# Jittor/PointCloudLib

Hardware: AMD Instinct MI355X
Metric: point-clouds/sec fwd+bwd, PointNet++ SSG B=32 N=1024 (higher is better)
Workload: dtype f32; 1 GPU; PointNet++ SSG cls train step (fwd+bwd+SGD), B=32/GPU, N=1024 xyz+normal, gauss_ball clouds (BASELINE configs[1]); global_batch=32, n_points=1024, parallelism=dp1, launch=eager, grad_overlap=False, cpu_affinity=numa node 0 (gpu0), 128 cpus, world_size=1, sync_bn=False, entry_points=per-stack (pcl_mlp_stack_*_f32)

## Files before the change

### pointcloudlib_amd/csrc/compact.hip

```cpp
#include "common.h"

namespace pcl {

struct GoffMulti { const int32_t* cnt[4]; int32_t* goff[4]; };
__device__ __forceinline__ void group_offsets_body(const int32_t* __restrict__ cnt, int G, int32_t* __restrict__ goff);
__global__ __launch_bounds__(1024) void group_offsets_kernel(const int32_t* __restrict__ cnt, int G, int32_t* __restrict__ goff) {
    group_offsets_body(cnt, G, goff);
}
__global__ __launch_bounds__(1024) void group_offsets_multi_kernel(const GoffMulti a, int G) {
    group_offsets_body(a.cnt[blockIdx.x], G, a.goff[blockIdx.x]);
}
__device__ __forceinline__ void group_offsets_body(const int32_t* __restrict__ cnt, int G, int32_t* __restrict__ goff) {
    __shared__ int tot[16];
    constexpr int U = 8;
    const int lane = threadIdx.x & 63, w = threadIdx.x >> 6;
    const int per = ((G + 15) / 16 + 63) / 64 * 64;
    const int lo = min(w * per, G), hi = min(lo + per, G);
    int s = 0;
    rows_in_flight<U>(cnt, 1, lo + lane, 64, hi, [&](int, int v) { s += max(v, 1); });
#pragma unroll
    for (int o = 32; o > 0; o >>= 1) s += __shfl_xor(s, o);
    if (lane == 0) tot[w] = s;
    __syncthreads();
    int run = 0, all = 0;
#pragma unroll
    for (int j = 0; j < 16; ++j) { const int t = tot[j]; run += j < w ? t : 0; all += t; }
    rows_in_flight<U>(lo, 64, hi, [&](int g0) { return max(cnt[min(g0 + lane, hi - 1)], 1); },
                      [&](int g0, int v) {
                          int inc = v;
#pragma unroll
                          for (int o = 1; o < 64; o <<= 1) { const int t = __shfl_up(inc, o); if (lane >= o) inc += t; }
                          if (g0 + lane < hi) goff[g0 + lane] = run + inc - v;
                          run += __shfl(inc, 63);
                      });
    if (threadIdx.x == 0) goff[G] = all;
}

__global__ __launch_bounds__(256) void group_compact_kernel(const float* __restrict__ xyz, const float* __restrict__ new_xyz,
                                                            const float* __restrict__ feat, const int32_t* __restrict__ idx,
                                                            const int32_t* __restrict__ cnt, const int32_t* __restrict__ goff,
                                                            int G, int N, int m, int ns, int C, int use_xyz, int S,
                                                            float* __restrict__ rows, int2* __restrict__ rmeta,
                                                            int32_t* __restrict__ rsrc) {
    const int g = blockIdx.x, wave = threadIdx.x >> 6, lane = threadIdx.x & 63;
    const int D = (use_xyz ? 3 : 0) + C, off3 = use_xyz ? 3 : 0;
    const int c = max(cnt[g], 1), base = goff[g];
    const int b = g / m;
    const int32_t* I = idx + (size_t)g * ns;
    const int chunk = (ns + 3) >> 2;
    const int s_lo = wave * chunk, s_hi = min(s_lo + chunk, c);
    if (s_lo >= s_hi) return;
    float* o = rows + (size_t)base * S;
    const float* fb = feat ? feat + (size_t)b * N * C : nullptr;
    if (C >= 32) {
        float q[3] = {0.f, 0.f, 0.f};
        if (use_xyz && lane < 3) q[0] = new_xyz[(size_t)g * 3 + lane];
        for (int s = s_lo; s < s_hi; s += 4) {
            int k[4];
#pragma unroll
            for (int j = 0; j < 4; ++j) k[j] = I[min(s + j, s_hi - 1)];
            for (int c0 = 0; c0 < C; c0 += 128) {
                float v[4][2];
#pragma unroll
                for (int j = 0; j < 4; ++j)
#pragma unroll
                    for (int h = 0; h < 2; ++h) {
                        const int ch = min(c0 + h * 64 + lane, C - 1);
                        v[j][h] = fb[(size_t)k[j] * C + ch];
                    }
#pragma unroll
                for (int j = 0; j < 4; ++j)
#pragma unroll
                    for (int h = 0; h < 2; ++h) {
                        const int ch = c0 + h * 64 + lane;
                        if (s + j < s_hi && ch < C) o[(size_t)(s + j) * S + off3 + ch] = v[j][h];
                    }
            }
            if (use_xyz && lane < 3) {
#pragma unroll
                for (int j = 0; j < 4; ++j)
                    if (s + j < s_hi) o[(size_t)(s + j) * S + lane] = __fsub_rn(xyz[((size_t)b * N + k[j]) * 3 + lane], q[0]);
            }
            if (lane < S - D) {
#pragma unroll
                for (int j = 0; j < 4; ++j)
                    if (s + j < s_hi) o[(size_t)(s + j) * S + D + lane] = 0.f;
            }
        }
    } else {
        for (int s = s_lo + lane; s < s_hi; s += 64) {
            const int k = I[s];
            float* oo = o + (size_t)s * S;
            if (use_xyz) {
#pragma unroll
                for (int d = 0; d < 3; ++d) oo[d] = __fsub_rn(xyz[((size_t)b * N + k) * 3 + d], new_xyz[(size_t)g * 3 + d]);
            }
            for (int d = 0; d < C; ++d) oo[off3 + d] = fb[(size_t)k * C + d];
            for (int d = D; d < S; ++d) oo[d] = 0.f;
        }
    }
    for (int s = s_lo + lane; s < s_hi; s += 64) {
        const int mult = s == 0 ? ns - c + 1 : 1;
        rmeta[base + s] = make_int2(g, s | (mult << 16));
        rsrc[base + s] = b * N + I[s];
    }
}

template <int V>
__global__ __launch_bounds__(256) void bn_act_max_rows_kernel(const float* __restrict__ Y, const int32_t* __restrict__ goff,
                                                              const float* __restrict__ scale, const float* __restrict__ shift,
                                                              float slope, int G, int C, float* __restrict__ out,
                                                              int32_t* __restrict__ arg, float* __restrict__ ymax) {
    const int CV = C / V;
    const size_t total = (size_t)G * CV;
    for (size_t e = (size_t)blockIdx.x * 256 + threadIdx.x; e < total; e += (size_t)gridDim.x * 256) {
        const size_t g = e / CV;
        const int c = (int)(e - g * CV) * V;
        float a[V], bsh[V], best[V], by[V];
        int bi[V];
#pragma unroll
        for (int v = 0; v < V; ++v) { a[v] = scale[c + v]; bsh[v] = shift[c + v]; best[v] = -INFINITY; by[v] = 0.f; bi[v] = 0; }
        const int r0 = goff[g], r1 = goff[g + 1];
        for (int r = r0; r < r1; r += 4) {
            float yy[4][V];
#pragma unroll
            for (int j = 0; j < 4; ++j) {
                const float* src = Y + (size_t)min(r + j, r1 - 1) * C + c;
                if constexpr (V == 4) {
                    const float4 t = *reinterpret_cast<const float4*>(src);
                    yy[j][0] = t.x; yy[j][1] = t.y; yy[j][2] = t.z; yy[j][3] = t.w;
                } else {
                    yy[j][0] = *src;
                }
            }
#pragma unroll
            for (int j = 0; j < 4; ++j) {
                if (r + j < r1) {
#pragma unroll
                    for (int v = 0; v < V; ++v) {
                        const float u = fmaf(a[v], yy[j][v], bsh[v]);
                        const float z = u > 0.f ? u : u * slope;
                        if (z > best[v]) { best[v] = z; bi[v] = r + j - r0; by[v] = yy[j][v]; }
                    }
                }
            }
        }
#pragma unroll
        for (int v = 0; v < V; ++v) { out[g * C + c + v] = best[v]; arg[g * C + c + v] = bi[v]; ymax[g * C + c + v] = by[v]; }
    }
}

__global__ __launch_bounds__(256) void scatter_rows_add_kernel(const float* __restrict__ grows, const int32_t* __restrict__ rsrc,
                                                               const int32_t* __restrict__ n_rows, int D, int off, int C,
                                                               float* __restrict__ gfeat) {
    const int n = *n_rows, lane = threadIdx.x & 63;
    const int wv = blockIdx.x * 4 + (threadIdx.x >> 6), nw = gridDim.x * 4;
    for (int r = wv * 2; r < n; r += nw * 2) {
        const int r2 = min(r + 1, n - 1);
        const size_t d0 = (size_t)rsrc[r] * C, d1 = (size_t)rsrc[r2] * C;
        for (int c = lane; c < C; c += 64) {
            const float v0 = grows[(size_t)r * D + off + c], v1 = grows[(size_t)r2 * D + off + c];
            unsafeAtomicAdd(&gfeat[d0 + c], v0);
            if (r + 1 < n) unsafeAtomicAdd(&gfeat[d1 + c], v1);
        }
    }
}

constexpr int GL_MAXH = 4;
constexpr int GL_RPI = 4;
constexpr int GL_CF = 4;

__device__ __forceinline__ float glin_row_value(float u, const float4& L, const float4& F, const float (&wx)[3], const float (&wf)[GL_CF]) {
    const float t = fmaf(wx[2], L.z, fmaf(wx[1], L.y, fmaf(wx[0], L.x, u)));
    return fmaf(wf[3], F.w, fmaf(wf[2], F.z, fmaf(wf[1], F.y, fmaf(wf[0], F.x, t))));
}

struct DenseJob { const float* src; float* dst; int rows, cols, ldw, first, blocks; };

__global__ __launch_bounds__(256) void group_rows_meta_kernel(const float* __restrict__ xyz, const float* __restrict__ new_xyz,
                                                              const float* __restrict__ fs, int CF,
                                                              const int32_t* __restrict__ idx, const int32_t* __restrict__ cnt,
                                                              const int32_t* __restrict__ goff, int G, int N, int m, int ns,
                                                              int2* __restrict__ rmeta, int32_t* __restrict__ rsrc,
                                                              float4* __restrict__ rloc, float4* __restrict__ rfeat, DenseJob dj) {
    if ((int)blockIdx.x >= dj.first) {
        const int n = dj.rows * dj.cols;
        for (int i = ((int)blockIdx.x - dj.first) * 256 + (int)threadIdx.x; i < n; i += dj.blocks * 256) {
            const int r = i / dj.cols;
            dj.dst[i] = dj.src[(size_t)r * dj.ldw + (i - r * dj.cols)];
        }
        return;
    }
    const int g = blockIdx.x * 4 + (threadIdx.x >> 6), lane = threadIdx.x & 63;
    if (g >= G) return;
    const int c = max(cnt[g], 1), base = goff[g], b = g / m;
    const int32_t* I = idx + (size_t)g * ns;
    float q0 = 0.f, q1 = 0.f, q2 = 0.f;
    if (xyz) { q0 = new_xyz[(size_t)g * 3]; q1 = new_xyz[(size_t)g * 3 + 1]; q2 = new_xyz[(size_t)g * 3 + 2]; }
    for (int s = lane; s < c; s += 64) {
        const int mult = s == 0 ? ns - c + 1 : 1;
        const int src = b * N + I[s];
        rmeta[base + s] = make_int2(g, s | (mult << 16));
        rsrc[base + s] = src;
        float4 L = make_float4(0.f, 0.f, 0.f, (float)mult);
        if (xyz) {
            const float* pk = xyz + (size_t)src * 3;
            L.x = __fsub_rn(pk[0], q0); L.y = __fsub_rn(pk[1], q1); L.z = __fsub_rn(pk[2], q2);
        }
        rloc[base + s] = L;
        if (rfeat) {
            float f[4] = {0.f, 0.f, 0.f, 0.f};
            for (int j = 0; j < CF; ++j) f[j] = fs[(size_t)src * CF + j];
            rfeat[base + s] = make_float4(f[0], f[1], f[2], f[3]);
        }
    }
}

template <int NH>
__global__ __launch_bounds__(256) void group_linear_kernel(const float* __restrict__ Uf, const float* __restrict__ Wx,
                                                           const float* __restrict__ Wfs, int CF, int ldw,
                                                           const float4* __restrict__ rloc, const float4* __restrict__ rfeat,
                                                           const int32_t* __restrict__ rsrc,
                                                           const int32_t* __restrict__ n_rows, int C1, float* __restrict__ Y,
                                                           double* __restrict__ stats) {
    __shared__ double red[2][4][64 * NH];
    const int wave = threadIdx.x >> 6, lane = threadIdx.x & 63;
    const int R = *n_rows;
    float wx[NH][3], wf[NH][GL_CF];
    double ss[NH], qq[NH];
#pragma unroll
    for (int h = 0; h < NH; ++h) {
        const int ch = lane + 64 * h;
#pragma unroll
        for (int d = 0; d < 3; ++d) wx[h][d] = (Wx && ch < C1) ? Wx[(size_t)ch * ldw + d] : 0.f;
#pragma unroll
        for (int f = 0; f < GL_CF; ++f) wf[h][f] = (f < CF && ch < C1) ? Wfs[(size_t)ch * ldw + f] : 0.f;
        ss[h] = 0.0; qq[h] = 0.0;
    }
    const int stride = gridDim.x * 4 * GL_RPI;
    int r0 = (blockIdx.x * 4 + wave) * GL_RPI;
    float4 nl[GL_RPI], nf[GL_RPI]; int sr[GL_RPI];
#pragma unroll
    for (int j = 0; j < GL_RPI; ++j) {
        const int r = min(r0 + j, R - 1);
        nl[j] = rloc[r]; sr[j] = Uf ? rsrc[r] : 0; nf[j] = CF ? rfeat[r] : make_float4(0.f, 0.f, 0.f, 0.f);
    }
    for (; r0 < R; r0 += stride) {
        float4 L[GL_RPI], F[GL_RPI]; int cs[GL_RPI];
#pragma unroll
        for (int j = 0; j < GL_RPI; ++j) { L[j] = nl[j]; F[j] = nf[j]; cs[j] = sr[j]; }
        {
            const int rn = r0 + stride;
#pragma unroll
            for (int j = 0; j < GL_RPI; ++j) {
                const int r = min(rn + j, R - 1);
                nl[j] = rloc[r]; sr[j] = Uf ? rsrc[r] : 0; nf[j] = CF ? rfeat[r] : make_float4(0.f, 0.f, 0.f, 0.f);
            }
        }
#pragma unroll
        for (int h = 0; h < NH; ++h) {
            const int ch = min(lane + 64 * h, C1 - 1);
            float u[GL_RPI];
#pragma unroll
            for (int j = 0; j < GL_RPI; ++j) u[j] = Uf ? Uf[(size_t)cs[j] * C1 + ch] : 0.f;
#pragma unroll
            for (int j = 0; j < GL_RPI; ++j) {
                if (r0 + j < R && lane + 64 * h < C1) {
                    const float y = glin_row_value(u[j], L[j], F[j], wx[h], wf[h]);
                    Y[(size_t)(r0 + j) * C1 + ch] = y;
                    const double w = (double)L[j].w;
                    ss[h] += w * (double)y; qq[h] += w * (double)y * (double)y;
                }
            }
        }
    }
#pragma unroll
    for (int h = 0; h < NH; ++h) { red[0][wave][lane + 64 * h] = ss[h]; red[1][wave][lane + 64 * h] = qq[h]; }
    __syncthreads();
    for (int ch = threadIdx.x; ch < C1; ch += 256) {
        double* dst = stats + (size_t)blockIdx.x * 2 * C1;
        dst[ch] = (red[0][0][ch] + red[0][1][ch]) + (red[0][2][ch] + red[0][3][ch]);
        dst[C1 + ch] = (red[1][0][ch] + red[1][1][ch]) + (red[1][2][ch] + red[1][3][ch]);
    }
}

template <int NH>
__global__ __launch_bounds__(256) void group_linear_bwd_kernel(const float4* __restrict__ rloc, const float4* __restrict__ rfeat,
                                                               int CF, const float* __restrict__ dU, const float* __restrict__ Y,
                                                               const float* __restrict__ a_, const float* __restrict__ k1_,
                                                               const float* __restrict__ k2_, const float* __restrict__ mu_,
                                                               const int32_t* __restrict__ rsrc,
                                                               const int32_t* __restrict__ n_rows, int C1, float* __restrict__ dUf,
                                                               float* __restrict__ dWx_part, float* __restrict__ dWf_part) {
    __shared__ float red[3 + GL_CF][4][64 * NH];
    const int wave = threadIdx.x >> 6, lane = threadIdx.x & 63;
    const int R = *n_rows;
    float a[NH], k1[NH], k2[NH], mu[NH], gw[NH][3 + GL_CF];
#pragma unroll
    for (int h = 0; h < NH; ++h) {
        const int ch = min(lane + 64 * h, C1 - 1);
        a[h] = a_[ch]; k1[h] = k1_[ch]; k2[h] = k2_[ch]; mu[h] = mu_[ch];
#pragma unroll
        for (int d = 0; d < 3 + GL_CF; ++d) gw[h][d] = 0.f;
    }
    const int stride = gridDim.x * 4 * GL_RPI;
    int r0 = (blockIdx.x * 4 + wave) * GL_RPI;
    float4 nl[GL_RPI], nf[GL_RPI]; int sr[GL_RPI];
#pragma unroll
    for (int j = 0; j < GL_RPI; ++j) {
        const int r = min(r0 + j, R - 1);
        nl[j] = rloc[r]; sr[j] = dUf ? rsrc[r] : 0; nf[j] = dWf_part ? rfeat[r] : make_float4(0.f, 0.f, 0.f, 0.f);
    }
    for (; r0 < R; r0 += stride) {
        float4 L[GL_RPI], F[GL_RPI]; int cs[GL_RPI];
#pragma unroll
        for (int j = 0; j < GL_RPI; ++j) { L[j] = nl[j]; F[j] = nf[j]; cs[j] = sr[j]; }
        {
            const int rn = r0 + stride;
#pragma unroll
            for (int j = 0; j < GL_RPI; ++j) {
                const int r = min(rn + j, R - 1);
                nl[j] = rloc[r]; sr[j] = dUf ? rsrc[r] : 0; nf[j] = dWf_part ? rfeat[r] : make_float4(0.f, 0.f, 0.f, 0.f);
            }
        }
#pragma unroll
        for (int h = 0; h < NH; ++h) {
            const int ch = min(lane + 64 * h, C1 - 1);
            float du[GL_RPI], y[GL_RPI];
#pragma unroll
            for (int j = 0; j < GL_RPI; ++j) {
                const size_t o = (size_t)min(r0 + j, R - 1) * C1 + ch;
                du[j] = dU[o]; y[j] = Y[o];
            }
#pragma unroll
            for (int j = 0; j < GL_RPI; ++j) {
                if (r0 + j < R && lane + 64 * h < C1) {
                    const float dy = fmaf(a[h], du[j], -L[j].w * fmaf(k2[h], y[j] - mu[h], k1[h]));
                    if (dUf) unsafeAtomicAdd(&dUf[(size_t)cs[j] * C1 + ch], dy);
                    gw[h][0] = fmaf(dy, L[j].x, gw[h][0]); gw[h][1] = fmaf(dy, L[j].y, gw[h][1]);
                    gw[h][2] = fmaf(dy, L[j].z, gw[h][2]);
                    gw[h][3] = fmaf(dy, F[j].x, gw[h][3]); gw[h][4] = fmaf(dy, F[j].y, gw[h][4]);
                    gw[h][5] = fmaf(dy, F[j].z, gw[h][5]); gw[h][6] = fmaf(dy, F[j].w, gw[h][6]);
                }
            }
        }
    }
    if (dWx_part || dWf_part) {
#pragma unroll
        for (int h = 0; h < NH; ++h)
#pragma unroll
            for (int d = 0; d < 3 + GL_CF; ++d) red[d][wave][lane + 64 * h] = gw[h][d];
        __syncthreads();
        if (dWx_part)
            for (int e = threadIdx.x; e < C1 * 3; e += 256) {
                const int ch = e / 3, d = e - ch * 3;
                dWx_part[(size_t)blockIdx.x * C1 * 3 + e] = (red[d][0][ch] + red[d][1][ch]) + (red[d][2][ch] + red[d][3][ch]);
            }
        if (dWf_part)
            for (int e = threadIdx.x; e < C1 * CF; e += 256) {
                const int ch = e / CF, d = 3 + (e - ch * CF);
                dWf_part[(size_t)blockIdx.x * C1 * CF + e] = (red[d][0][ch] + red[d][1][ch]) + (red[d][2][ch] + red[d][3][ch]);
            }
    }
}

__device__ __forceinline__ void glin_load_weights(const float* __restrict__ Wx, const float* __restrict__ Wfs, int CF, int ldw, int c4,
                                                  float (&wx)[4][3], float (&wf)[4][GL_CF]) {
#pragma unroll
    for (int v = 0; v < 4; ++v) {
#pragma unroll
        for (int d = 0; d < 3; ++d) wx[v][d] = Wx ? Wx[(size_t)(c4 + v) * ldw + d] : 0.f;
#pragma unroll
        for (int f = 0; f < GL_CF; ++f) wf[v][f] = f < CF ? Wfs[(size_t)(c4 + v) * ldw + f] : 0.f;
    }
}
template <int LPR>
__global__ __launch_bounds__(256) void group_linear_v4_kernel(const float* __restrict__ Uf, const float* __restrict__ Wx,
                                                              const float* __restrict__ Wfs, int CF, int ldw,
                                                              const float4* __restrict__ rloc, const float4* __restrict__ rfeat,
                                                              const int32_t* __restrict__ rsrc,
                                                              const int32_t* __restrict__ n_rows, float* __restrict__ Y,
                                                              double* __restrict__ stats) {
    constexpr int C1 = 4 * LPR, RPW = 64 / LPR, U = 4;
    __shared__ double red[2][4][C1];
    const int wave = threadIdx.x >> 6, lane = threadIdx.x & 63;
    const int cl = lane % LPR, rsub = lane / LPR, c4 = 4 * cl;
    const int R = *n_rows;
    float wx[4][3], wf[4][GL_CF];
    double ss[4], qq[4];
#pragma unroll
    for (int v = 0; v < 4; ++v) {
#pragma unroll
        for (int d = 0; d < 3; ++d) wx[v][d] = Wx ? Wx[(size_t)(c4 + v) * ldw + d] : 0.f;
#pragma unroll
        for (int f = 0; f < GL_CF; ++f) wf[v][f] = f < CF ? Wfs[(size_t)(c4 + v) * ldw + f] : 0.f;
        ss[v] = 0.0; qq[v] = 0.0;
    }
    const int stride = gridDim.x * 4 * RPW * U;
    for (int r0 = (blockIdx.x * 4 + wave) * RPW * U; r0 < R; r0 += stride) {
        float4 L[U], F[U], u[U];
#pragma unroll
        for (int j = 0; j < U; ++j) {
            const int r = min(r0 + j * RPW + rsub, R - 1);
            L[j] = rloc[r];
            F[j] = CF ? rfeat[r] : make_float4(0.f, 0.f, 0.f, 0.f);
            u[j] = Uf ? *reinterpret_cast<const float4*>(Uf + (size_t)rsrc[r] * C1 + c4) : make_float4(0.f, 0.f, 0.f, 0.f);
        }
#pragma unroll
        for (int j = 0; j < U; ++j) {
            const int r = r0 + j * RPW + rsub;
            if (r < R) {
                float y[4] = {u[j].x, u[j].y, u[j].z, u[j].w};
                const double w = (double)L[j].w;
#pragma unroll
                for (int v = 0; v < 4; ++v) {
                    const float t = glin_row_value(y[v], L[j], F[j], wx[v], wf[v]);
                    y[v] = t;
                    ss[v] += w * (double)t; qq[v] += w * (double)t * (double)t;
                }
                *reinterpret_cast<float4*>(Y + (size_t)r * C1 + c4) = make_float4(y[0], y[1], y[2], y[3]);
            }
        }
    }
#pragma unroll
    for (int v = 0; v < 4; ++v) {
#pragma unroll
        for (int off = LPR; off < 64; off <<= 1) { ss[v] += __shfl_xor(ss[v], off); qq[v] += __shfl_xor(qq[v], off); }
        if (rsub == 0) { red[0][wave][c4 + v] = ss[v]; red[1][wave][c4 + v] = qq[v]; }
    }
    __syncthreads();
    for (int ch = threadIdx.x; ch < C1; ch += 256) {
        double* dst = stats + (size_t)blockIdx.x * 2 * C1;
        dst[ch] = (red[0][0][ch] + red[0][1][ch]) + (red[0][2][ch] + red[0][3][ch]);
        dst[C1 + ch] = (red[1][0][ch] + red[1][1][ch]) + (red[1][2][ch] + red[1][3][ch]);
    }
}

template <int LPR>
__global__ __launch_bounds__(256) void group_linear_bwd_v4_kernel(const float4* __restrict__ rloc, const float4* __restrict__ rfeat,
                                                                  int CF, const float* __restrict__ dU, const float* __restrict__ Y,
                                                                  const float* __restrict__ a_, const float* __restrict__ k1_,
                                                                  const float* __restrict__ k2_, const float* __restrict__ mu_,
                                                                  const int32_t* __restrict__ rsrc,
                                                                  const int32_t* __restrict__ n_rows, float* __restrict__ dUf,
                                                                  float* __restrict__ dWx_part, float* __restrict__ dWf_part) {
    constexpr int C1 = 4 * LPR, RPW = 64 / LPR, U = 4;
    __shared__ float red[3 + GL_CF][4][C1];
    const int wave = threadIdx.x >> 6, lane = threadIdx.x & 63;
    const int cl = lane % LPR, rsub = lane / LPR, c4 = 4 * cl;
    const int R = *n_rows;
    float a[4], k1[4], k2[4], mu[4], gw[3 + GL_CF][4];
#pragma unroll
    for (int v = 0; v < 4; ++v) {
        a[v] = a_[c4 + v]; k1[v] = k1_[c4 + v]; k2[v] = k2_[c4 + v]; mu[v] = mu_[c4 + v];
#pragma unroll
        for (int d = 0; d < 3 + GL_CF; ++d) gw[d][v] = 0.f;
    }
    const int stride = gridDim.x * 4 * RPW * U;
    for (int r0 = (blockIdx.x * 4 + wave) * RPW * U; r0 < R; r0 += stride) {
        float4 L[U], F[U], du[U], yv[U];
        int src[U];
#pragma unroll
        for (int j = 0; j < U; ++j) {
            const int r = min(r0 + j * RPW + rsub, R - 1);
            L[j] = rloc[r];
            F[j] = dWf_part ? rfeat[r] : make_float4(0.f, 0.f, 0.f, 0.f);
            src[j] = dUf ? rsrc[r] : 0;
            du[j] = *reinterpret_cast<const float4*>(dU + (size_t)r * C1 + c4);
            yv[j] = *reinterpret_cast<const float4*>(Y + (size_t)r * C1 + c4);
        }
#pragma unroll
        for (int j = 0; j < U; ++j) {
            const int r = r0 + j * RPW + rsub;
            if (r < R) {
                const float dd[4] = {du[j].x, du[j].y, du[j].z, du[j].w}, yy[4] = {yv[j].x, yv[j].y, yv[j].z, yv[j].w};
#pragma unroll
                for (int v = 0; v < 4; ++v) {
                    const float dy = fmaf(a[v], dd[v], -L[j].w * fmaf(k2[v], yy[v] - mu[v], k1[v]));
                    if (dUf) unsafeAtomicAdd(&dUf[(size_t)src[j] * C1 + c4 + v], dy);
                    gw[0][v] = fmaf(dy, L[j].x, gw[0][v]); gw[1][v] = fmaf(dy, L[j].y, gw[1][v]); gw[2][v] = fmaf(dy, L[j].z, gw[2][v]);
                    gw[3][v] = fmaf(dy, F[j].x, gw[3][v]); gw[4][v] = fmaf(dy, F[j].y, gw[4][v]);
                    gw[5][v] = fmaf(dy, F[j].z, gw[5][v]); gw[6][v] = fmaf(dy, F[j].w, gw[6][v]);
                }
            }
        }
    }
    if (dWx_part || dWf_part) {
#pragma unroll
        for (int d = 0; d < 3 + GL_CF; ++d)
#pragma unroll
            for (int v = 0; v < 4; ++v) {
                float t = gw[d][v];
#pragma unroll
                for (int off = LPR; off < 64; off <<= 1) t += __shfl_xor(t, off);
                if (rsub == 0) red[d][wave][c4 + v] = t;
            }
        __syncthreads();
        if (dWx_part)
            for (int e = threadIdx.x; e < C1 * 3; e += 256) {
                const int ch = e / 3, d = e - ch * 3;
                dWx_part[(size_t)blockIdx.x * C1 * 3 + e] = (red[d][0][ch] + red[d][1][ch]) + (red[d][2][ch] + red[d][3][ch]);
            }
        if (dWf_part)
            for (int e = threadIdx.x; e < C1 * CF; e += 256) {
                const int ch = e / CF, d = 3 + (e - ch * CF);
                dWf_part[(size_t)blockIdx.x * C1 * CF + e] = (red[d][0][ch] + red[d][1][ch]) + (red[d][2][ch] + red[d][3][ch]);
            }
    }
}

template <int LPR>
__global__ __launch_bounds__(256) void group_linear_bwd_regen_kernel(const float4* __restrict__ rloc, const float4* __restrict__ rfeat,
                                                                     const float* __restrict__ Wx, const float* __restrict__ Wfs, int CF,
                                                                     int ldw, const float* __restrict__ dU, const float* __restrict__ a_,
                                                                     const float* __restrict__ k1_, const float* __restrict__ k2_,
                                                                     const float* __restrict__ mu_, const int32_t* __restrict__ n_rows,
                                                                     float* __restrict__ dWx_part, float* __restrict__ dWf_part) {
    constexpr int C1 = 4 * LPR, RPW = 64 / LPR, CH = 4, U = 3;
    __shared__ float red[3 + GL_CF][4][C1];
    const int wave = threadIdx.x >> 6, lane = threadIdx.x & 63;
    const int cl = lane % LPR, rsub = lane / LPR, c4 = 4 * cl;
    const int R = *n_rows;
    float wx[4][3], wf[4][GL_CF];
    float a[4], k1[4], k2[4], mu[4], gw[3 + GL_CF][4];
    glin_load_weights(Wx, Wfs, CF, ldw, c4, wx, wf);
#pragma unroll
    for (int v = 0; v < 4; ++v) {
        a[v] = a_[c4 + v]; k1[v] = k1_[c4 + v]; k2[v] = k2_[c4 + v]; mu[v] = mu_[c4 + v];
#pragma unroll
        for (int d = 0; d < 3 + GL_CF; ++d) gw[d][v] = 0.f;
    }
    const int stride = gridDim.x * 4 * RPW * CH, base = (blockIdx.x * 4 + wave) * RPW * CH;
    for (int t0 = 0; base + (t0 / CH) * stride < R; t0 += U) {
        float4 L[U], F[U], du[U];
        int row[U];
#pragma unroll
        for (int j = 0; j < U; ++j) {
            const int t = t0 + j;
            row[j] = base + (t / CH) * stride + (t % CH) * RPW + rsub;
            const int r = min(row[j], R - 1);
            L[j] = rloc[r];
            F[j] = CF ? rfeat[r] : make_float4(0.f, 0.f, 0.f, 0.f);
            du[j] = *reinterpret_cast<const float4*>(dU + (size_t)r * C1 + c4);
        }
#pragma unroll
        for (int j = 0; j < U; ++j) {
            if (row[j] < R) {
                const float dd[4] = {du[j].x, du[j].y, du[j].z, du[j].w};
#pragma unroll
                for (int v = 0; v < 4; ++v) {
                    const float y = glin_row_value(0.f, L[j], F[j], wx[v], wf[v]);
                    const float dy = fmaf(a[v], dd[v], -L[j].w * fmaf(k2[v], y - mu[v], k1[v]));
                    gw[0][v] = fmaf(dy, L[j].x, gw[0][v]); gw[1][v] = fmaf(dy, L[j].y, gw[1][v]); gw[2][v] = fmaf(dy, L[j].z, gw[2][v]);
                    gw[3][v] = fmaf(dy, F[j].x, gw[3][v]); gw[4][v] = fmaf(dy, F[j].y, gw[4][v]);
                    gw[5][v] = fmaf(dy, F[j].z, gw[5][v]); gw[6][v] = fmaf(dy, F[j].w, gw[6][v]);
                }
            }
        }
    }
#pragma unroll
    for (int d = 0; d < 3 + GL_CF; ++d)
#pragma unroll
        for (int v = 0; v < 4; ++v) {
            float t = gw[d][v];
#pragma unroll
            for (int off = LPR; off < 64; off <<= 1) t += __shfl_xor(t, off);
            if (rsub == 0) red[d][wave][c4 + v] = t;
        }
    __syncthreads();
    if (dWx_part)
        for (int e = threadIdx.x; e < C1 * 3; e += 256) {
            const int ch = e / 3, d = e - ch * 3;
            dWx_part[(size_t)blockIdx.x * C1 * 3 + e] = (red[d][0][ch] + red[d][1][ch]) + (red[d][2][ch] + red[d][3][ch]);
        }
// ... 192 lines not shown
    __syncthreads();
    int run = inc - s;
    for (int w = 0; w < wave; ++w) run += wtot[w];
    for (int i = i0; i < i1; ++i) {
        const int t = off[i];
        off[i] = run;
        int pos = run;
        for (int w = 0; w < RT_W; ++w) { const int c = cnt[w * N + i]; cnt[w * N + i] = pos; pos += c; }
        run += t;
    }
    if (tid == 0) off[N] = re - rb;
    __syncthreads();
    for (int g = g0; g < g1; ++g) {
        const int q0 = group_off[g_first + g], q1 = group_off[g_first + g + 1];
        for (int r = q0 + lane; r < q1; r += 64) lst[atomicAdd(&mycnt[rsrc[r] - pbase], 1)] = r;
        __builtin_amdgcn_fence(__ATOMIC_SEQ_CST, "wavefront");
        __builtin_amdgcn_wave_barrier();
    }
    __syncthreads();
    for (int pl = tid; pl < N; pl += RT_T) in_off[pbase + pl] = rb + off[pl];
    if (b == B - 1 && tid == 0) in_off[pbase + N] = re;
    for (int i = tid; i < re - rb; i += RT_T) in_rows[rb + i] = lst[i];
}

__global__ __launch_bounds__(256) void group_linear_dw_kernel(const float* __restrict__ px, const float* __restrict__ pf, int rows,
                                                              int C1, int CF, int off, int ld, float* __restrict__ dW0) {
    const int nx = px ? C1 * 3 : 0, nf = pf ? C1 * CF : 0;
    const int e = blockIdx.x * 4 + (threadIdx.x >> 6), lane = threadIdx.x & 63;
    if (e >= nx + nf) return;
    const bool isx = e < nx;
    const float* src = isx ? px + e : pf + (e - nx);
    const int n = isx ? nx : nf;
    float s = 0.f;
    rows_in_flight<8>(src, n, lane, 64, rows, [&](int, float v) { s += v; });
#pragma unroll
    for (int o = 32; o > 0; o >>= 1) s += __shfl_xor(s, o);
    if (lane == 0) {
        if (isx) dW0[(size_t)(e / 3) * ld + e % 3] = s;
        else dW0[(size_t)((e - nx) / CF) * ld + off + (e - nx) % CF] = s;
    }
}

}
using namespace pcl;

extern "C" int pcl_group_offsets_i32(const int32_t* cnt, int G, int32_t* group_off, void* stream) {
    PCL_REQUIRE(cnt && group_off && G >= 1, "pcl_group_offsets_i32: bad arguments");
    hipLaunchKernelGGL(group_offsets_kernel, dim3(1), dim3(1024), 0, as_stream(stream), cnt, G, group_off);
    return check_launch("pcl_group_offsets_i32");
}

extern "C" int pcl_group_offsets_multi_i32(int n, const int32_t* const* cnt, int G, int32_t* const* group_off, void* stream) {
    PCL_REQUIRE(cnt && group_off && G >= 1 && n >= 1 && n <= 4, "pcl_group_offsets_multi_i32: bad arguments (n = %d: 1..4)", n);
    GoffMulti a = {};
    for (int i = 0; i < n; ++i) {
        PCL_REQUIRE(cnt[i] && group_off[i], "pcl_group_offsets_multi_i32: null array %d", i);
        a.cnt[i] = cnt[i]; a.goff[i] = group_off[i];
    }
    hipLaunchKernelGGL(group_offsets_multi_kernel, dim3(n), dim3(1024), 0, as_stream(stream), a, G);
    return check_launch("pcl_group_offsets_multi_i32");
}

extern "C" int pcl_group_compact_f32(const float* xyz, const float* new_xyz, const float* feat, const int32_t* idx,
                                     const int32_t* cnt, const int32_t* group_off, int B, int N, int m, int ns, int C,
                                     int use_xyz, int row_stride, float* rows, int32_t* row_meta, int32_t* row_src,
                                     void* stream) {
    PCL_REQUIRE(idx && cnt && rows && row_meta && row_src && group_off, "pcl_group_compact_f32: null pointer");
    PCL_REQUIRE(!use_xyz || (xyz && new_xyz), "pcl_group_compact_f32: use_xyz needs xyz and new_xyz");
    PCL_REQUIRE(C == 0 || feat, "pcl_group_compact_f32: C=%d needs feat", C);
    PCL_REQUIRE(B >= 1 && N >= 1 && m >= 1 && ns >= 1 && ns < 32768 && C >= 0 && (use_xyz || C > 0), "pcl_group_compact_f32: bad sizes");
    const int D = (use_xyz ? 3 : 0) + C;
    PCL_REQUIRE(row_stride >= D && row_stride < D + 64, "pcl_group_compact_f32: row_stride=%d for %d columns", row_stride, D);
    const int G = B * m;
    hipLaunchKernelGGL(group_compact_kernel, dim3(G), dim3(256), 0, as_stream(stream), xyz, new_xyz, feat, idx, cnt, group_off, G, N, m,
                       ns, C, use_xyz, row_stride, rows, reinterpret_cast<int2*>(row_meta), row_src);
    return check_launch("pcl_group_compact_f32");
}

extern "C" int pcl_bn_act_max_rows_f32(const float* Y, const int32_t* group_off, const float* scale, const float* shift,
                                       float slope, int G, int C, float* out, int32_t* arg, float* ymax, void* stream) {
    PCL_REQUIRE(Y && group_off && scale && shift && out && arg && ymax && G >= 1 && C >= 1, "pcl_bn_act_max_rows_f32: bad arguments");
    const bool vec = (C % 4 == 0) && al16(Y);
    const size_t total = (size_t)G * (vec ? C / 4 : C);
    int blocks = (int)((total + 255) / 256);
    if (blocks > 16384) blocks = 16384;
    if (vec)
        hipLaunchKernelGGL(bn_act_max_rows_kernel<4>, dim3(blocks), dim3(256), 0, as_stream(stream), Y, group_off, scale, shift, slope,
                           G, C, out, arg, ymax);
    else
        hipLaunchKernelGGL(bn_act_max_rows_kernel<1>, dim3(blocks), dim3(256), 0, as_stream(stream), Y, group_off, scale, shift, slope,
                           G, C, out, arg, ymax);
    return check_launch("pcl_bn_act_max_rows_f32");
}

extern "C" int pcl_scatter_rows_add_f32(const float* grows, const int32_t* row_src, const int32_t* n_rows_dev, int rows_cap,
                                        int D, int off, int C, int n_dst_rows, float* gfeat, void* stream) {
    PCL_REQUIRE(grows && row_src && n_rows_dev && gfeat && rows_cap >= 1 && D >= 1 && off >= 0 && C >= 1 && off + C <= D && n_dst_rows >= 1,
                "pcl_scatter_rows_add_f32: bad arguments");
    hipStream_t st = as_stream(stream);
    hipError_t e = hipMemsetAsync(gfeat, 0, sizeof(float) * (size_t)n_dst_rows * C, st);
    if (e != hipSuccess) return fail(PCL_EHIP, "pcl_scatter_rows_add_f32: memset: %s", hipGetErrorString(e));
    size_t blocks = ((size_t)rows_cap + 7) / 8;
    if (blocks > 8192) blocks = 8192;
    hipLaunchKernelGGL(scatter_rows_add_kernel, dim3((int)blocks), dim3(256), 0, st, grows, row_src, n_rows_dev, D, off, C, gfeat);
    return check_launch("pcl_scatter_rows_add_f32");
}

constexpr int GL_BLOCKS = 1024;

extern "C" int pcl_group_linear_stat_rows(int B, int m) { return (B < 1 || m < 1) ? 0 : GL_BLOCKS; }

namespace pcl {
int group_linear_fwd_impl(const float* xyz, const float* new_xyz, const float* Uf, const float* Wx, const float* feat_small,
                          const float* Wf_small, int CF, int ldw, const int32_t* idx, const int32_t* cnt, const int32_t* group_off, int B,
                          int N, int m, int ns, int C1, float* Y, int32_t* row_meta, int32_t* row_src, float* row_loc, float* row_feat,
                          double* stats_ws, void* stream, int phase, const float* dense_src, float* dense_dst, int dense_cols);
}
extern "C" int pcl_group_linear_f32(const float* xyz, const float* new_xyz, const float* Uf, const float* Wx, const float* feat_small,
                                    const float* Wf_small, int CF, int ldw, const int32_t* idx, const int32_t* cnt,
                                    const int32_t* group_off, int B, int N, int m, int ns, int C1, float* Y, int32_t* row_meta,
                                    int32_t* row_src, float* row_loc, float* row_feat, double* stats_ws, void* stream) {
    return group_linear_fwd_impl(xyz, new_xyz, Uf, Wx, feat_small, Wf_small, CF, ldw, idx, cnt, group_off, B, N, m, ns, C1, Y, row_meta, row_src,
                                 row_loc, row_feat, stats_ws, stream, 3, nullptr, nullptr, 0);
}
int pcl::group_linear_fwd_impl(const float* xyz, const float* new_xyz, const float* Uf, const float* Wx, const float* feat_small,
                               const float* Wf_small, int CF, int ldw, const int32_t* idx, const int32_t* cnt, const int32_t* group_off,
                               int B, int N, int m, int ns, int C1, float* Y, int32_t* row_meta, int32_t* row_src, float* row_loc,
                               float* row_feat, double* stats_ws, void* stream, int phase, const float* dense_src, float* dense_dst,
                               int dense_cols) {
    PCL_REQUIRE(idx && cnt && group_off && Y && row_meta && row_src && row_loc && stats_ws, "pcl_group_linear_f32: null pointer");
    PCL_REQUIRE(CF == 0 || row_feat, "pcl_group_linear_f32: inline features need row_feat");
    PCL_REQUIRE(phase == 1 || Uf || Wx || CF > 0, "pcl_group_linear_f32: need features (Uf or feat_small) and/or coordinates (Wx)");
    PCL_REQUIRE(CF >= 0 && CF <= GL_CF && (CF == 0 || (feat_small && Wf_small)), "pcl_group_linear_f32: CF=%d inline features (<= %d)", CF, GL_CF);
    PCL_REQUIRE(!Wx || (xyz && new_xyz), "pcl_group_linear_f32: Wx needs xyz and new_xyz");
    PCL_REQUIRE(ldw >= (Wx ? 3 : 0) && ldw >= CF, "pcl_group_linear_f32: ldw=%d", ldw);
    PCL_REQUIRE(B >= 1 && N >= 1 && m >= 1 && ns >= 1 && ns < 32768 && C1 >= 1 && C1 <= 64 * GL_MAXH,
                "pcl_group_linear_f32: bad sizes B=%d N=%d m=%d ns=%d C1=%d (C1 <= %d)", B, N, m, ns, C1, 64 * GL_MAXH);
    const int G = B * m;
    hipStream_t st = as_stream(stream);
    if (phase & 1) {
        const int gb = (G + 3) / 4;
        DenseJob dj = {dense_src, dense_dst, C1, dense_cols, ldw, gb, 0};
        if (dense_dst) dj.blocks = (C1 * dense_cols + 1023) / 1024 < 64 ? (C1 * dense_cols + 1023) / 1024 : 64;
        hipLaunchKernelGGL(group_rows_meta_kernel, dim3(gb + dj.blocks), dim3(256), 0, st, Wx ? xyz : nullptr, new_xyz, feat_small, CF, idx, cnt,
                           group_off, G, N, m, ns, reinterpret_cast<int2*>(row_meta), row_src, reinterpret_cast<float4*>(row_loc),
                           reinterpret_cast<float4*>(CF ? row_feat : nullptr), dj);
        int rc = check_launch("pcl_group_linear_f32(meta)");
        if (rc || phase == 1) return rc;
    }
    const float4* rl = reinterpret_cast<const float4*>(row_loc);
    const float4* rf = reinterpret_cast<const float4*>(row_feat);
    const dim3 grid(GL_BLOCKS), block(256);
    if (al16(Y, Uf) && (C1 == 64 || C1 == 128 || C1 == 256)) {
        if (C1 == 64) hipLaunchKernelGGL(group_linear_v4_kernel<16>, grid, block, 0, st, Uf, Wx, Wf_small, CF, ldw, rl, rf, row_src, group_off + G, Y, stats_ws);
        else if (C1 == 128) hipLaunchKernelGGL(group_linear_v4_kernel<32>, grid, block, 0, st, Uf, Wx, Wf_small, CF, ldw, rl, rf, row_src, group_off + G, Y, stats_ws);
        else hipLaunchKernelGGL(group_linear_v4_kernel<64>, grid, block, 0, st, Uf, Wx, Wf_small, CF, ldw, rl, rf, row_src, group_off + G, Y, stats_ws);
        return check_launch("pcl_group_linear_f32");
    }
    if (C1 <= 64) hipLaunchKernelGGL(group_linear_kernel<1>, grid, block, 0, st, Uf, Wx, Wf_small, CF, ldw, rl, rf, row_src, group_off + G, C1, Y, stats_ws);
    else if (C1 <= 128) hipLaunchKernelGGL(group_linear_kernel<2>, grid, block, 0, st, Uf, Wx, Wf_small, CF, ldw, rl, rf, row_src, group_off + G, C1, Y, stats_ws);
    else hipLaunchKernelGGL(group_linear_kernel<4>, grid, block, 0, st, Uf, Wx, Wf_small, CF, ldw, rl, rf, row_src, group_off + G, C1, Y, stats_ws);
    return check_launch("pcl_group_linear_f32");
}

namespace pcl {
int group_linear_bwd_impl(const float* row_loc, const float* row_feat, int CF, const float* dU, const float* Y, const float* a,
                          const float* k1, const float* k2, const float* mu, const int32_t* row_src, const int32_t* n_rows_dev, int B, int N,
                          int C1, float* dUf, float* dWx_part, float* dWf_part, float* dW0, int ldw, int off, void* stream, bool duf_is_zero);
}
extern "C" int pcl_group_linear_bwd_f32(const float* row_loc, const float* row_feat, int CF, const float* dU, const float* Y,
                                        const float* a, const float* k1, const float* k2, const float* mu, const int32_t* row_src,
                                        const int32_t* n_rows_dev, int B, int N, int C1, float* dUf, float* dWx_part,
                                        float* dWf_part, float* dW0, int ldw, int off, void* stream) {
    return group_linear_bwd_impl(row_loc, row_feat, CF, dU, Y, a, k1, k2, mu, row_src, n_rows_dev, B, N, C1, dUf, dWx_part, dWf_part, dW0, ldw,
                                 off, stream, false);
}
int pcl::group_linear_bwd_impl(const float* row_loc, const float* row_feat, int CF, const float* dU, const float* Y, const float* a,
                               const float* k1, const float* k2, const float* mu, const int32_t* row_src, const int32_t* n_rows_dev, int B,
                               int N, int C1, float* dUf, float* dWx_part, float* dWf_part, float* dW0, int ldw, int off, void* stream,
                               bool duf_is_zero) {
    PCL_REQUIRE(row_loc && dU && Y && a && k1 && k2 && mu && row_src && n_rows_dev, "pcl_group_linear_bwd_f32: null pointer");
    PCL_REQUIRE(dUf || dWx_part || dWf_part, "pcl_group_linear_bwd_f32: nothing to compute");
    PCL_REQUIRE(!dWf_part || (row_feat && CF >= 1 && CF <= GL_CF), "pcl_group_linear_bwd_f32: dWf needs row_feat, CF=%d", CF);
    PCL_REQUIRE(B >= 1 && N >= 1 && C1 >= 1 && C1 <= 64 * GL_MAXH, "pcl_group_linear_bwd_f32: bad sizes");
    PCL_REQUIRE(!dW0 || ((dWx_part || dWf_part) && ldw >= (dWx_part ? 3 : 0) && off >= 0 && ldw >= off + (dWf_part ? CF : 0)),
                "pcl_group_linear_bwd_f32: dW0 needs the partial buffers and ldw=%d >= off=%d + CF", ldw, off);
    hipStream_t st = as_stream(stream);
    if (dUf && !duf_is_zero) {
        hipError_t e = hipMemsetAsync(dUf, 0, sizeof(float) * (size_t)B * N * C1, st);
        if (e != hipSuccess) return fail(PCL_EHIP, "pcl_group_linear_bwd_f32: memset: %s", hipGetErrorString(e));
    }
    const float4* rl = reinterpret_cast<const float4*>(row_loc);
    const float4* rf = reinterpret_cast<const float4*>(row_feat);
    const dim3 grid(GL_BLOCKS), block(256);
    if (!dUf && al16(Y, dU) && (C1 == 64 || C1 == 128 || C1 == 256)) {
        if (C1 == 64) hipLaunchKernelGGL(group_linear_bwd_v4_kernel<16>, grid, block, 0, st, rl, rf, CF, dU, Y, a, k1, k2, mu, row_src, n_rows_dev, dUf, dWx_part, dWf_part);
        else if (C1 == 128) hipLaunchKernelGGL(group_linear_bwd_v4_kernel<32>, grid, block, 0, st, rl, rf, CF, dU, Y, a, k1, k2, mu, row_src, n_rows_dev, dUf, dWx_part, dWf_part);
        else hipLaunchKernelGGL(group_linear_bwd_v4_kernel<64>, grid, block, 0, st, rl, rf, CF, dU, Y, a, k1, k2, mu, row_src, n_rows_dev, dUf, dWx_part, dWf_part);
    } else if (C1 <= 64) hipLaunchKernelGGL(group_linear_bwd_kernel<1>, grid, block, 0, st, rl, rf, CF, dU, Y, a, k1, k2, mu, row_src, n_rows_dev, C1, dUf, dWx_part, dWf_part);
    else if (C1 <= 128) hipLaunchKernelGGL(group_linear_bwd_kernel<2>, grid, block, 0, st, rl, rf, CF, dU, Y, a, k1, k2, mu, row_src, n_rows_dev, C1, dUf, dWx_part, dWf_part);
    else hipLaunchKernelGGL(group_linear_bwd_kernel<4>, grid, block, 0, st, rl, rf, CF, dU, Y, a, k1, k2, mu, row_src, n_rows_dev, C1, dUf, dWx_part, dWf_part);
    int rc = check_launch("pcl_group_linear_bwd_f32");
    if (rc || !dW0) return rc;
    const int n = (dWx_part ? C1 * 3 : 0) + (dWf_part ? C1 * CF : 0);
    hipLaunchKernelGGL(group_linear_dw_kernel, dim3((n + 3) / 4), block, 0, st, dWx_part, dWf_part, GL_BLOCKS, C1, CF, off, ldw, dW0);
    return check_launch("pcl_group_linear_bwd_f32(dW)");
}

extern "C" int pcl_group_linear_dw_sum_f32(const float* dWx_part, const float* dWf_part, int rows, int C1, int CF, int off, int ld, float* dW0,
                                           void* stream) {
    PCL_REQUIRE((dWx_part || dWf_part) && dW0 && rows >= 1 && C1 >= 1, "pcl_group_linear_dw_sum_f32: bad arguments");
    PCL_REQUIRE(!dWf_part || CF >= 1, "pcl_group_linear_dw_sum_f32: dWf_part needs CF >= 1");
    PCL_REQUIRE(ld >= (dWx_part ? 3 : 0) && off >= 0 && ld >= off + (dWf_part ? CF : 0), "pcl_group_linear_dw_sum_f32: ld=%d below off=%d + CF", ld, off);
    const int n = (dWx_part ? C1 * 3 : 0) + (dWf_part ? C1 * CF : 0);
    hipLaunchKernelGGL(group_linear_dw_kernel, dim3((n + 3) / 4), dim3(256), 0, as_stream(stream), dWx_part, dWf_part, rows, C1, CF, off, ld, dW0);
    return check_launch("pcl_group_linear_dw_sum_f32");
}

extern "C" int pcl_group_rows_transpose_supported(int N, int m, int ns) {
    return N >= 1 && m >= 1 && ns >= 1 && ((size_t)(RT_W + 1) * N + 1 + (size_t)m * ns) * 4 <= 150 * 1024;
}
extern "C" int pcl_group_rows_transpose_i32(const int32_t* row_src, const int32_t* group_off, int B, int N, int m, int ns, int32_t* in_off,
                                            int32_t* in_rows, void* stream) {
    PCL_REQUIRE(row_src && group_off && in_off && in_rows && B >= 1 && m >= 1 && ns >= 1, "pcl_group_rows_transpose_i32: bad arguments");
    PCL_REQUIRE(pcl_group_rows_transpose_supported(N, m, ns), "pcl_group_rows_transpose_i32: N=%d m=%d ns=%d beyond the LDS-resident form", N, m, ns);
    const size_t lds = ((size_t)(RT_W + 1) * N + 1 + (size_t)m * ns) * 4;
    auto kern = rows_transpose_kernel;
    if (int rc = lds_opt_in(kern, lds, "pcl_group_rows_transpose_i32")) return rc;
    hipLaunchKernelGGL(kern, dim3(B), dim3(RT_T), lds, as_stream(stream), row_src, group_off, m, N, B, in_off, in_rows);
    return check_launch("pcl_group_rows_transpose_i32");
}
extern "C" int pcl_group_linear_bwd_gather_supported(int C1) { return g_lab.scatter_gather && (C1 == 64 || C1 == 128 || C1 == 256); }
extern "C" int pcl_group_linear_bwd_gather_f32(const float* row_loc, const float* dU, const float* Y, const float* a, const float* k1,
                                               const float* k2, const float* mu, const int32_t* in_off, const int32_t* in_rows, int B, int N,
                                               int C1, float* dUf, float* dWx_part, float* dW0, int ldw, void* stream) {
    PCL_REQUIRE(row_loc && dU && Y && a && k1 && k2 && mu && in_off && in_rows && dUf, "pcl_group_linear_bwd_gather_f32: null pointer");
    PCL_REQUIRE(B >= 1 && N >= 1 && pcl_group_linear_bwd_gather_supported(C1), "pcl_group_linear_bwd_gather_f32: bad sizes (C1 = %d: 64, 128 or 256)", C1);
    PCL_REQUIRE(al16(dU, Y, dUf), "pcl_group_linear_bwd_gather_f32: 16-byte aligned rows");
    PCL_REQUIRE(!dW0 || (dWx_part && ldw >= 3), "pcl_group_linear_bwd_gather_f32: dW0 needs dWx_part and ldw >= 3");
    hipStream_t st = as_stream(stream);
    const float4* rl = reinterpret_cast<const float4*>(row_loc);
    const dim3 grid(GL_BLOCKS), block(256);
    const int P = B * N;
    if (C1 == 64) hipLaunchKernelGGL(group_linear_bwd_gather_kernel<16>, grid, block, 0, st, rl, dU, Y, a, k1, k2, mu, in_off, in_rows, P, dUf, dWx_part);
    else if (C1 == 128) hipLaunchKernelGGL(group_linear_bwd_gather_kernel<32>, grid, block, 0, st, rl, dU, Y, a, k1, k2, mu, in_off, in_rows, P, dUf, dWx_part);
    else hipLaunchKernelGGL(group_linear_bwd_gather_kernel<64>, grid, block, 0, st, rl, dU, Y, a, k1, k2, mu, in_off, in_rows, P, dUf, dWx_part);
    int rc = check_launch("pcl_group_linear_bwd_gather_f32");
    if (rc || !dW0) return rc;
    hipLaunchKernelGGL(group_linear_dw_kernel, dim3((C1 * 3 + 3) / 4), block, 0, st, dWx_part, (const float*)nullptr, GL_BLOCKS, C1, 0, 0, ldw, dW0);
    return check_launch("pcl_group_linear_bwd_gather_f32(dW)");
}

extern "C" int pcl_group_linear_bwd_regen_supported(int C1, int CF) {
    return (C1 == 64 || C1 == 128 || C1 == 256) && CF >= 0 && CF <= GL_CF;
}
extern "C" int pcl_group_linear_bwd_regen_f32(const float* row_loc, const float* row_feat, const float* Wx, const float* Wf_small, int CF,
                                              int ldw, const float* dU, const float* a, const float* k1, const float* k2, const float* mu,
                                              const int32_t* n_rows_dev, int C1, float* dWx_part, float* dWf_part, float* dW0, int ld0, int off,
                                              void* stream) {
    PCL_REQUIRE(row_loc && dU && a && k1 && k2 && mu && n_rows_dev, "pcl_group_linear_bwd_regen_f32: null pointer");
    PCL_REQUIRE(pcl_group_linear_bwd_regen_supported(C1, CF), "pcl_group_linear_bwd_regen_f32: C1 = %d (64, 128 or 256), CF = %d (<= %d)", C1, CF, GL_CF);
    PCL_REQUIRE(Wx || CF > 0, "pcl_group_linear_bwd_regen_f32: need the forward's weights (Wx and/or Wf_small)");
    PCL_REQUIRE(CF == 0 || (row_feat && Wf_small), "pcl_group_linear_bwd_regen_f32: CF=%d inline features need row_feat and Wf_small", CF);
    PCL_REQUIRE(ldw >= (Wx ? 3 : 0) && ldw >= CF, "pcl_group_linear_bwd_regen_f32: ldw=%d", ldw);
    PCL_REQUIRE(dWx_part || dWf_part, "pcl_group_linear_bwd_regen_f32: nothing to compute");
    PCL_REQUIRE(!dWf_part || CF >= 1, "pcl_group_linear_bwd_regen_f32: dWf_part needs CF >= 1");
    PCL_REQUIRE(al16(dU, row_loc, row_feat), "pcl_group_linear_bwd_regen_f32: 16-byte aligned rows");
    PCL_REQUIRE(!dW0 || (ld0 >= (dWx_part ? 3 : 0) && off >= 0 && ld0 >= off + (dWf_part ? CF : 0)),
                "pcl_group_linear_bwd_regen_f32: dW0 needs ld0=%d >= off=%d + CF", ld0, off);
    hipStream_t st = as_stream(stream);
    const float4* rl = reinterpret_cast<const float4*>(row_loc);
    const float4* rf = reinterpret_cast<const float4*>(row_feat);
    const dim3 grid(GL_BLOCKS), block(256);
    if (C1 == 64) hipLaunchKernelGGL(group_linear_bwd_regen_kernel<16>, grid, block, 0, st, rl, rf, Wx, Wf_small, CF, ldw, dU, a, k1, k2, mu, n_rows_dev, dWx_part, dWf_part);
    else if (C1 == 128) hipLaunchKernelGGL(group_linear_bwd_regen_kernel<32>, grid, block, 0, st, rl, rf, Wx, Wf_small, CF, ldw, dU, a, k1, k2, mu, n_rows_dev, dWx_part, dWf_part);
    else hipLaunchKernelGGL(group_linear_bwd_regen_kernel<64>, grid, block, 0, st, rl, rf, Wx, Wf_small, CF, ldw, dU, a, k1, k2, mu, n_rows_dev, dWx_part, dWf_part);
    int rc = check_launch("pcl_group_linear_bwd_regen_f32");
    if (rc || !dW0) return rc;
    const int n = (dWx_part ? C1 * 3 : 0) + (dWf_part ? C1 * CF : 0);
    hipLaunchKernelGGL(group_linear_dw_kernel, dim3((n + 3) / 4), block, 0, st, dWx_part, dWf_part, GL_BLOCKS, C1, CF, off, ld0, dW0);
    return check_launch("pcl_group_linear_bwd_regen_f32(dW)");
}
extern "C" int pcl_group_linear_bwd_gather_regen_f32(const float* row_loc, const float* dU, const float* Uf, const float* Wx, int ldw,
                                                     const float* a, const float* k1, const float* k2, const float* mu, const int32_t* in_off,
                                                     const int32_t* in_rows, int B, int N, int C1, float* dUf, float* dWx_part, float* dW0,
                                                     int ld0, void* stream) {
    PCL_REQUIRE(row_loc && dU && Uf && a && k1 && k2 && mu && in_off && in_rows && dUf, "pcl_group_linear_bwd_gather_regen_f32: null pointer");
    PCL_REQUIRE(B >= 1 && N >= 1 && pcl_group_linear_bwd_gather_supported(C1), "pcl_group_linear_bwd_gather_regen_f32: bad sizes (C1 = %d: 64, 128 or 256)", C1);
    PCL_REQUIRE(al16(dU, Uf, dUf, row_loc) && al16(a, k1, k2, mu), "pcl_group_linear_bwd_gather_regen_f32: 16-byte aligned rows");
    PCL_REQUIRE(!Wx || ldw >= 3, "pcl_group_linear_bwd_gather_regen_f32: ldw=%d", ldw);
    PCL_REQUIRE(!dW0 || (dWx_part && ld0 >= 3), "pcl_group_linear_bwd_gather_regen_f32: dW0 needs dWx_part and ld0 >= 3");
    hipStream_t st = as_stream(stream);
    const float4* rl = reinterpret_cast<const float4*>(row_loc);
    const dim3 grid(GL_BLOCKS), block(256);
    const int P = B * N;
    if (C1 == 64) hipLaunchKernelGGL(group_linear_bwd_gather_regen_kernel<16>, grid, block, 0, st, rl, dU, Uf, Wx, ldw, a, k1, k2, mu, in_off, in_rows, P, dUf, dWx_part);
    else if (C1 == 128) hipLaunchKernelGGL(group_linear_bwd_gather_regen_kernel<32>, grid, block, 0, st, rl, dU, Uf, Wx, ldw, a, k1, k2, mu, in_off, in_rows, P, dUf, dWx_part);
    else hipLaunchKernelGGL(group_linear_bwd_gather_regen_kernel<64>, grid, block, 0, st, rl, dU, Uf, Wx, ldw, a, k1, k2, mu, in_off, in_rows, P, dUf, dWx_part);
    int rc = check_launch("pcl_group_linear_bwd_gather_regen_f32");
    if (rc || !dW0) return rc;
    hipLaunchKernelGGL(group_linear_dw_kernel, dim3((C1 * 3 + 3) / 4), block, 0, st, dWx_part, (const float*)nullptr, GL_BLOCKS, C1, 0, 0, ld0, dW0);
    return check_launch("pcl_group_linear_bwd_gather_regen_f32(dW)");
}
```

Baseline: 18390 point-clouds/s.

## Software-pipeline row loads in group-linear and bn-max kernels, specialize on Uf/CF

The group_linear_v4 kernel becomes a software pipeline: the next stride's row loads and the index prefetch two strides ahead are issued while the current rows are computed, with sched barriers and empty asm fences keeping that order. It is also templated on whether Uf and CF are present, which removes runtime branches and dead loads. bn_act_max_rows now uses the rows_in_flight helper to keep several row loads outstanding. The aim is to hide global-memory latency in these gather-heavy kernels, at the cost of more register pressure and extra tail handling.

```diff
diff --git a/pointcloudlib_amd/csrc/compact.hip b/pointcloudlib_amd/csrc/compact.hip
--- a/pointcloudlib_amd/csrc/compact.hip
+++ b/pointcloudlib_amd/csrc/compact.hip
@@ -106,6 +106,14 @@
     }
 }
 
+constexpr int MAXROWS_U = 4;
+__device__ __forceinline__ void loaded_fence(float& v) { asm volatile("" : "+v"(v) : : "memory"); }
+__device__ __forceinline__ void loaded_fence(float4& v) {
+    typedef float f32x4 __attribute__((ext_vector_type(4)));
+    f32x4 t = {v.x, v.y, v.z, v.w};
+    asm volatile("" : "+v"(t) : : "memory");
+    v = make_float4(t.x, t.y, t.z, t.w);
+}
 template <int V>
 __global__ __launch_bounds__(256) void bn_act_max_rows_kernel(const float* __restrict__ Y, const int32_t* __restrict__ goff,
                                                               const float* __restrict__ scale, const float* __restrict__ shift,
@@ -121,30 +129,24 @@
 #pragma unroll
         for (int v = 0; v < V; ++v) { a[v] = scale[c + v]; bsh[v] = shift[c + v]; best[v] = -INFINITY; by[v] = 0.f; bi[v] = 0; }
         const int r0 = goff[g], r1 = goff[g + 1];
-        for (int r = r0; r < r1; r += 4) {
-            float yy[4][V];
-#pragma unroll
-            for (int j = 0; j < 4; ++j) {
-                const float* src = Y + (size_t)min(r + j, r1 - 1) * C + c;
-                if constexpr (V == 4) {
-                    const float4 t = *reinterpret_cast<const float4*>(src);
-                    yy[j][0] = t.x; yy[j][1] = t.y; yy[j][2] = t.z; yy[j][3] = t.w;
-                } else {
-                    yy[j][0] = *src;
+        const float* col = Y + c;
+        rows_in_flight<MAXROWS_U>(r0, 1, r1,
+            [&](int q) {
+                if constexpr (V == 4) return *reinterpret_cast<const float4*>(col + (size_t)q * C);
+                else return col[(size_t)q * C];
+            },
+            [&](int q, auto t) {
+                loaded_fence(t);
+                float yy[V];
+                if constexpr (V == 4) { yy[0] = t.x; yy[1] = t.y; yy[2] = t.z; yy[3] = t.w; }
+                else yy[0] = t;
+#pragma unroll
+                for (int v = 0; v < V; ++v) {
+                    const float u = fmaf(a[v], yy[v], bsh[v]);
+                    const float z = u > 0.f ? u : u * slope;
+                    if (z > best[v]) { best[v] = z; bi[v] = q - r0; by[v] = yy[v]; }
                 }
-            }
-#pragma unroll
-            for (int j = 0; j < 4; ++j) {
-                if (r + j < r1) {
-#pragma unroll
-                    for (int v = 0; v < V; ++v) {
-                        const float u = fmaf(a[v], yy[j][v], bsh[v]);
-                        const float z = u > 0.f ? u : u * slope;
-                        if (z > best[v]) { best[v] = z; bi[v] = r + j - r0; by[v] = yy[j][v]; }
-                    }
-                }
-            }
-        }
+            });
 #pragma unroll
         for (int v = 0; v < V; ++v) { out[g * C + c + v] = best[v]; arg[g * C + c + v] = bi[v]; ymax[g * C + c + v] = by[v]; }
     }
@@ -374,7 +376,13 @@
         for (int f = 0; f < GL_CF; ++f) wf[v][f] = f < CF ? Wfs[(size_t)(c4 + v) * ldw + f] : 0.f;
     }
 }
-template <int LPR>
+__device__ __forceinline__ void glin_take(float4& v) {
+    typedef float f32x4 __attribute__((ext_vector_type(4)));
+    f32x4 t = {v.x, v.y, v.z, v.w};
+    asm volatile("" : "+v"(t));
+    v = make_float4(t.x, t.y, t.z, t.w);
+}
+template <int LPR, bool UF, bool CFX>
 __global__ __launch_bounds__(256) void group_linear_v4_kernel(const float* __restrict__ Uf, const float* __restrict__ Wx,
                                                               const float* __restrict__ Wfs, int CF, int ldw,
                                                               const float4* __restrict__ rloc, const float4* __restrict__ rfeat,
@@ -388,38 +396,58 @@
     const int R = *n_rows;
     float wx[4][3], wf[4][GL_CF];
     double ss[4], qq[4];
-#pragma unroll
-    for (int v = 0; v < 4; ++v) {
-#pragma unroll
-        for (int d = 0; d < 3; ++d) wx[v][d] = Wx ? Wx[(size_t)(c4 + v) * ldw + d] : 0.f;
-#pragma unroll
-        for (int f = 0; f < GL_CF; ++f) wf[v][f] = f < CF ? Wfs[(size_t)(c4 + v) * ldw + f] : 0.f;
-        ss[v] = 0.0; qq[v] = 0.0;
-    }
+    glin_load_weights(Wx, Wfs, CFX ? CF : 0, ldw, c4, wx, wf);
+#pragma unroll
+    for (int v = 0; v < 4; ++v) { ss[v] = 0.0; qq[v] = 0.0; }
     const int stride = gridDim.x * 4 * RPW * U;
-    for (int r0 = (blockIdx.x * 4 + wave) * RPW * U; r0 < R; r0 += stride) {
+    int r0 = (blockIdx.x * 4 + wave) * RPW * U;
+    if (r0 < R) {
+        const float4 Z4 = make_float4(0.f, 0.f, 0.f, 0.f);
         float4 L[U], F[U], u[U];
+        int sn[U];
+        auto row_of = [&](int base, int j) { return min(base + j * RPW + rsub, R - 1); };
+        auto fill = [&](int j, int r) {
+            L[j] = rloc[r];
+            F[j] = CFX ? rfeat[r] : Z4;
+            u[j] = UF ? *reinterpret_cast<const float4*>(Uf + (size_t)sn[j] * C1 + c4) : Z4;
+        };
+        auto row = [&](int j, int r) {
+            float4 Lj = L[j], Fj = F[j], uj = u[j];
+            glin_take(Lj); if (CFX) glin_take(Fj); if (UF) glin_take(uj);
+            float y[4] = {uj.x, uj.y, uj.z, uj.w};
+            const double w = (double)Lj.w;
+#pragma unroll
+            for (int v = 0; v < 4; ++v) {
+                const float t = glin_row_value(y[v], Lj, Fj, wx[v], wf[v]);
+                y[v] = t;
+                ss[v] += w * (double)t; qq[v] += w * (double)t * (double)t;
+            }
+            *reinterpret_cast<float4*>(Y + (size_t)r * C1 + c4) = make_float4(y[0], y[1], y[2], y[3]);
+        };
+#pragma unroll
+        for (int j = 0; j < U; ++j) sn[j] = UF ? rsrc[row_of(r0, j)] : 0;
 #pragma unroll
         for (int j = 0; j < U; ++j) {
-            const int r = min(r0 + j * RPW + rsub, R - 1);
-            L[j] = rloc[r];
-            F[j] = CF ? rfeat[r] : make_float4(0.f, 0.f, 0.f, 0.f);
-            u[j] = Uf ? *reinterpret_cast<const float4*>(Uf + (size_t)rsrc[r] * C1 + c4) : make_float4(0.f, 0.f, 0.f, 0.f);
-        }
-#pragma unroll
-        for (int j = 0; j < U; ++j) {
-            const int r = r0 + j * RPW + rsub;
-            if (r < R) {
-                float y[4] = {u[j].x, u[j].y, u[j].z, u[j].w};
-                const double w = (double)L[j].w;
-#pragma unroll
-                for (int v = 0; v < 4; ++v) {
-                    const float t = glin_row_value(y[v], L[j], F[j], wx[v], wf[v]);
-                    y[v] = t;
-                    ss[v] += w * (double)t; qq[v] += w * (double)t * (double)t;
-                }
-                *reinterpret_cast<float4*>(Y + (size_t)r * C1 + c4) = make_float4(y[0], y[1], y[2], y[3]);
-            }
+            fill(j, row_of(r0, j));
+            if (UF) sn[j] = rsrc[row_of(r0 + stride, j)];
+        }
+        auto trip = [&]() {
+#pragma unroll
+            for (int j = 0; j < U; ++j) {
+                row(j, r0 + j * RPW + rsub);
+                fill(j, row_of(r0 + stride, j));
+                if (UF) sn[j] = __hip_atomic_load(rsrc + row_of(r0 + 2 * stride, j), __ATOMIC_RELAXED, __HIP_MEMORY_SCOPE_WAVEFRONT);
+                __builtin_amdgcn_sched_barrier(0);
+            }
+        };
+        if (r0 + U * RPW <= R) {
+            trip();
+            for (r0 += stride; r0 + U * RPW <= R; r0 += stride) trip();
+        }
+        if (r0 < R) {
+#pragma unroll
+            for (int j = 0; j < U; ++j)
+                if (r0 + j * RPW + rsub < R) row(j, r0 + j * RPW + rsub);
         }
     }
 #pragma unroll
@@ -918,9 +946,17 @@
     const float4* rf = reinterpret_cast<const float4*>(row_feat);
     const dim3 grid(GL_BLOCKS), block(256);
     if (al16(Y, Uf) && (C1 == 64 || C1 == 128 || C1 == 256)) {
-        if (C1 == 64) hipLaunchKernelGGL(group_linear_v4_kernel<16>, grid, block, 0, st, Uf, Wx, Wf_small, CF, ldw, rl, rf, row_src, group_off + G, Y, stats_ws);
-        else if (C1 == 128) hipLaunchKernelGGL(group_linear_v4_kernel<32>, grid, block, 0, st, Uf, Wx, Wf_small, CF, ldw, rl, rf, row_src, group_off + G, Y, stats_ws);
-        else hipLaunchKernelGGL(group_linear_v4_kernel<64>, grid, block, 0, st, Uf, Wx, Wf_small, CF, ldw, rl, rf, row_src, group_off + G, Y, stats_ws);
+        auto launch = [&](auto kernel) {
+            hipLaunchKernelGGL(kernel, grid, block, 0, st, Uf, Wx, Wf_small, CF, ldw, rl, rf, row_src, group_off + G, Y, stats_ws);
+        };
+        auto pick = [&](auto lpr) {
+            constexpr int LPR = decltype(lpr)::value;
+            if (Uf) { if (CF) launch(group_linear_v4_kernel<LPR, true, true>); else launch(group_linear_v4_kernel<LPR, true, false>); }
+            else { if (CF) launch(group_linear_v4_kernel<LPR, false, true>); else launch(group_linear_v4_kernel<LPR, false, false>); }
+        };
+        if (C1 == 64) pick(std::integral_constant<int, 16>());
+        else if (C1 == 128) pick(std::integral_constant<int, 32>());
+        else pick(std::integral_constant<int, 64>());
         return check_launch("pcl_group_linear_f32");
     }
     if (C1 <= 64) hipLaunchKernelGGL(group_linear_kernel<1>, grid, block, 0, st, Uf, Wx, Wf_small, CF, ldw, rl, rf, row_src, group_off + G, C1, Y, stats_ws);
```

Result: no change. 18380 point-clouds/s (-0.1%).
